# zilliztech/knowhere

Measured on AMD Instinct MI355X. Metric: QPS at recall@10>=0.95, IVF-PQ 100M x d=128 batch=10k, higher is better.
Workload: dtype f32

## Files before the change

### knowhere_amd/csrc/kernels.h

```cpp
#pragma once

#include <hip/hip_runtime.h>
#include <stdint.h>
#include <algorithm>
#include "sq_codec.h"

namespace knhip {

struct KnItem {
    int32_t list;
    int32_t npair;
    int64_t pair0;
};
struct KnPair {
    int32_t q;
    int32_t slot;
};

__host__ __device__ constexpr int pq_stream_phase(int lane) {
    const int l = lane & 31;
    return l < 4 ? l : l < 12 ? l + 4 : l < 16 ? l - 8 : l < 20 ? l - 16 : l < 28 ? l - 12 : l - 24;
}
constexpr int PQ_STREAM_PHASES = 16;
__host__ __device__ constexpr uint32_t pq_stream_mask(int j) {
    uint32_t m = 0;
    for (int l = 0; l < 32; l++) {
        if (pq_stream_phase(l) <= j) {
            m |= 1u << l;
        }
    }
    return m;
}
// ... 228 lines not shown
    P8Rec* pq_recs;
    const uint4* pq_codes_i;
    const void* pq_qi;
    const float* pq_qis;
    P16Rec* pq_recs16;
    int32_t* pq_ctr;
    int32_t pq_prune_mu;
    const void* pq_cb16;
    const void* pq_qh16;
    const float* pq_qd;
    const float* pq_sc;
    const float* pq_psum_s;
    unsigned char* pq_spill;
    int32_t pq_spill_cap;
    int32_t pq_spill_wgs;
    const int2* pq_unit_tiles;
};

int64_t pq_stream16r_blocks(int64_t len);
hipError_t launch_pq_stream16r(const uint8_t* codes, const int64_t* list_row_off, const int64_t* list_len,
                               const int64_t* list_sblk_off, int64_t nlist, uint4* out, hipStream_t s);
hipError_t launch_pq_psum(const uint8_t* codes, const int64_t* list_row_off, const int64_t* list_len,
                          const int64_t* list_sblk_off, int64_t nlist, const float* precomp_t, float* psum,
                          uint32_t* pabs_max_bits, hipStream_t s);
hipError_t launch_pqf_query_table(const float* queries, const float4* cb_m, int d, int64_t nq, bool is_l2, float pabs_max,
                                  void* qh, float* qs, hipStream_t s);
hipError_t launch_pqf_predict(const float* dump, int64_t stride, const int32_t* n_row, const float* gthr, const float* qs,
                              const float* qs2, const int64_t* keys, int nprobe, int64_t nlist, const int64_t* list_len,
                              int64_t nq, int cap, int k, bool is_l2, int32_t* poor, hipStream_t s);
size_t pqf_smem();
hipError_t launch_pq_stream16i(const uint8_t* codes, const int64_t* list_row_off, const int64_t* list_len,
// ... 60 lines not shown
hipError_t launch_pq_scan_q4(const PqScanArgs& a, bool is_l2, int64_t items_bound, hipStream_t s);
hipError_t launch_pq_cb_transpose(const float* cb, int M, int dsub, float4* cb_t, hipStream_t s);

int mscan_queries_per_unit(int kind, bool sample);
size_t mscan_flat_smem(int nstep);
size_t mscan_sq8_smem(int nstep, int bits = 8);
int mscan_finish_pmax(int cap, int k);
int mscan_sample_rows();
hipError_t launch_ms_block_norms(const float4* rows, int64_t total_blk, int nchunk, float* out, float* out_max,
                                 hipStream_t s, int row_type = KN_ROW_FP32);
hipError_t launch_ms_sq8_norms(const uint4* rows, int64_t total_blk, int nchunk16, int d, const float* trained,
                               float* out, float* out_max, hipStream_t s, int bits = 8);
hipError_t launch_ms_units(const int32_t* list_count_v, const int64_t* list_pair_off_v, int64_t nlist, int qt,
                           int64_t* unit_off, int64_t* nunits, KnItem* units, const int64_t* list_len,
                           int64_t code_size, double* unit_bytes, hipStream_t s, int cost_cap = 0,
                           int2* unit_tiles = nullptr);
inline int64_t ms_units_cost_bound(int64_t npairs, int qt, int64_t nlist, int64_t ntotal, int64_t max_len, int cost_cap) {
    const int64_t groups = npairs / qt + std::min<int64_t>(nlist, npairs) + 1;
    if (cost_cap <= 0) {
        return groups;
    }
    const int64_t max_ntile = std::max<int64_t>((max_len + 31) / 32, 1);
    const int64_t by_cost = groups + (2 * max_ntile * (npairs / 32 + groups) + cost_cap - 1) / cost_cap;
    const int64_t by_tiles = npairs / qt * max_ntile + ntotal / 32 + 2 * nlist + 1;
    return std::max<int64_t>(groups, std::min<int64_t>(by_cost, by_tiles));
}
hipError_t launch_mscan_flat(const MScanArgs& a, bool is_l2, int64_t units_bound, hipStream_t s);
int mscan_flat_bf16_qt(int nstep);
size_t mscan_flat_bf16_smem(int nstep);
hipError_t launch_mscan_flat_bf16(const MScanArgs& a, bool is_l2, int64_t units_bound, hipStream_t s);
hipError_t launch_mscan_sq8(const MScanArgs& a, bool is_l2, int64_t units_bound, hipStream_t s);
// ... 285 lines not shown
```

### knowhere_amd/csrc/knhip_api_search.hip

```cpp
#include "knhip_internal.h"

namespace knhip_host {

template <class A>
static A scan_args(const knhip_index* idx, const Workspace* ws, const Batch& b) {
    A a{};
    a.list_len = idx->d_list_len.as<int64_t>();
    a.list_row_off = idx->d_list_row_off.as<int64_t>();
    a.ids = idx->ids.as<int64_t>();
    a.d = idx->d;
    a.queries = b.q;
    a.bitset = b.bitset;
    a.bitset_nbits = b.nbits;
    a.partial_d = ws->partial_d.as<float>();
    a.partial_i = ws->partial_i.as<int64_t>();
    a.k = b.k;
    return a;
}
template <class A>
static A item_scan_args(const knhip_index* idx, const Workspace* ws, const Batch& b, const WorkTable& wt) {
    A a = scan_args<A>(idx, ws, b);
    a.items = wt.items;
    a.pairs = wt.pairs;
    a.nitems_dev = wt.nitems;
// ... 567 lines not shown
        HIP_TRY(ws->pq_recs16.reserve((size_t)std::max<int64_t>(std::max(plan.ms_units_bound, plan.ms_bound0), plan.npairs) *
                                      sizeof(P16Rec)));
        m.pq_codes_r = idx->rows_r.as<uint4>();
        m.pq_codes_i = idx->rows_i.as<uint4>();
        m.pq_qi = ws->ms_qi.p;
        m.pq_qis = ws->ms_qis.as<float>();
        m.pq_recs16 = ws->pq_recs16.as<P16Rec>();
    }
    if (f->form == 3) {
        f->qt = PD_QT;
        if (env.pqd_unit_cost > 0) {
            f->pqd_cost = env.pqd_unit_cost;
            f->pqd_bound = round_up(ms_units_cost_bound(plan.npairs, PD_QT, idx->nlist, idx->ntotal, idx->max_list_len,
                                                        f->pqd_cost), 8);
            HIP_TRY(ws->ms_units.reserve((size_t)f->pqd_bound * sizeof(KnItem)));
            HIP_TRY(ws->pqd_tiles.reserve((size_t)f->pqd_bound * sizeof(int2)));
            m.units = ws->ms_units.as<KnItem>();
            m.pq_unit_tiles = ws->pqd_tiles.as<int2>();
        }
        m.pq_cb16 = idx->pqd_cb16.p;
        m.pq_qh16 = ws->ms_qh16.p;
        m.pq_qd = ws->ms_qd.as<float>();
        m.pq_sc = idx->pqd_st.as<float>();
        m.pq_psum_s = idx->psum_s.as<float>();
        m.pq_spill_cap = 4 * 8192;
        if (idx->pqd_spill_cap > 0) {
            m.pq_spill_cap = idx->pqd_spill_cap;
        }
        m.pq_spill_wgs = 512;
        int dev = 0, ncu = 0;
        (void)hipGetDevice(&dev);
        if (hipDeviceGetAttribute(&ncu, hipDeviceAttributeMultiprocessorCount, dev) == hipSuccess && ncu > 0) {
            m.pq_spill_wgs = ncu;
// ... 93 lines not shown
}

int ms_group_units(const knhip_index* idx, Workspace* ws, const SearchPlan& plan, const Batch& b, const PqForm& f,
                   const WorkTable& wside, SideJoin* sj, hipStream_t s, MScanArgs& m) {
    const int64_t nlist = idx->nlist;
    StageTimer t(idx, s, KNHIP_STAGE_GROUP);
    if (sj->forked) {
        if (int rc = sj->join()) return rc;
    } else {
        HIP_TRY(launch_build_worktable(b.keys, b.nq, b.nprobe, nlist, plan.qg, plan.qg, idx->d_list_len.as<int64_t>(),
                                       idx->dev_code_size(), wside, s, -1));
    }
    m.pairs = wside.pairs;
    HIP_TRY(launch_ms_units(wside.list_count + nlist, wside.list_pair_off + nlist, nlist, f.qt, ws->ms_unit_off.as<int64_t>(),
                            ws->ms_nunits.as<int64_t>(), ws->ms_units.as<KnItem>(), idx->d_list_len.as<int64_t>(), idx->dev_code_size(),
                            idx->scan_bytes_dev.as<double>() + 2, s, f.pqd_cost, ws->pqd_tiles.as<int2>()));
    return KNHIP_OK;
}

int rows_exact_scan(const knhip_index* idx, Workspace* ws, const Batch& b, const WorkTable& wt, int64_t grid, bool one_pair,
                    hipStream_t s) {
    if (idx->desc.kind == KNHIP_IVF_FLAT) {
        FlatScanArgs a = flat_scan_args(idx, ws, b, wt);
        a.item_loop = one_pair;
        HIP_TRY(launch_flat_scan(a, idx->is_l2, false, grid, s, one_pair));
    } else {
        SqScanArgs a = sq_scan_args(idx, ws, b, wt);
        a.item_loop = one_pair;
        HIP_TRY(launch_sq_scan(a, idx->is_l2, grid, s, one_pair));
    }
    return KNHIP_OK;
// ... 30 lines not shown
    if (f.form == 2) {
        mf.pq_qs = m.pq_qis;
        mf.pq_prune_mu = 1;
    }
    if (f.form == 3) {
        mf.pq_qs = m.pq_qd;
    }
    HIP_TRY(launch_mscan_finish(mf, kind, is_l2, b.keys, b.cdis, nprobe, k, b.out_d, b.out_i, counters, 1, s));
    HIP_TRY(launch_ms_flag_pairs(m.overflow, 2, b.keys, nq, nprobe, nlist, idx->d_list_len.as<int64_t>(), k, wt.items, wt.pairs,
                                 wt.nitems, nullptr, s));
    MScanArgs r = m;
    r.pairs = wt.pairs;
    r.units = wt.items;
    r.nunits_dev = wt.nitems;
    r.unit_loop = 1;
    r.pq_unit_tiles = nullptr;
    r.ghist = nullptr;
    r.gmeta = nullptr;
    HIP_TRY(launch_filter(idx, plan, f, r, plan.npairs, s));
    HIP_TRY(launch_mscan_finish(mf, kind, is_l2, b.keys, b.cdis, nprobe, k, b.out_d, b.out_i, counters, 2, s));
    HIP_TRY(launch_ms_flag_pairs(m.overflow, 1, b.keys, nq, nprobe, nlist, idx->d_list_len.as<int64_t>(), k, wt.items, wt.pairs,
                                 wt.nitems, ws->partial_i.as<int64_t>(), s));
    if (int rc = exact_one_pair_items(idx, ws, plan, b, wt, s)) return rc;
    HIP_TRY(launch_merge_partials(ws->partial_d.as<float>(), ws->partial_i.as<int64_t>(), nq, nprobe, k, (int64_t)nprobe * k, k,
                                  is_l2, b.out_d, b.out_i, s, m.overflow));
    return KNHIP_OK;
}

int run_prefilter(const knhip_index* idx, Workspace* ws, const SearchPlan& plan, const Batch& b, const EnvSearch& env,
                  const WorkTable& wt, hipStream_t s, PqForm* f) {
    MScanArgs m;
// ... 155 lines not shown
```

### knowhere_amd/csrc/knhip_internal.h

```cpp
#pragma once
#include "../../include/knhip.h"
#include "common.h"
#include "kernels.h"
#include "knhip_env.h"

#include <cstdio>
#include <cstdlib>
#include <cstring>
#include <map>
#include <memory>
#include <mutex>
#include <numeric>
#include <random>
#include <string>
#include <vector>

using namespace knhip;

namespace knhip_host {

int fail(int code, const std::string& msg);

#define HIP_TRY(expr)                                                                              \
    do {                                                                                           \
// ... 100 lines not shown
    DevBuf recs4;
    DevBuf q4_ctr;
    DevBuf ghist;
    DevBuf gmeta;
    WorkTableBufs wt[2];
    DevBuf ms_qi, ms_qis, ms_qmu, pq_recs16;
    DevBuf rs_ovf;
    DevBuf ms_eps_max;
    DevBuf ms_cand_pess;
    DevBuf ms_units, ms_unit_off, ms_nunits, ms_cand, ms_cand_cnt;
    DevBuf ms_sample_off, ms_nrow;
    DevBuf ms_qh, ms_ql, ms_qs;
    DevBuf pq_recs, pq_ctr;
    DevBuf bf_kth;
    DevBuf ms_qh16, ms_qd, pq_spill;
    DevBuf pqd_tiles;
    DevBuf rs_sort;
    DevBuf h_queries, h_bitset, h_out_d, h_out_i, h_ref_d, h_ref_i;
    DevBuf tie_d, tie_i, tie_flag, tie_q, tie_r, tie_keys, tie_cdis;
    DevBuf tie_arr_d, tie_arr_i, tie_arr_n;
    DevBuf lk_plan, lk_scratch;
    std::mutex mu;
    hipStream_t side = nullptr;
    hipEvent_t ev_fork = nullptr, ev_join = nullptr;
    volatile int32_t* h_word = nullptr;
    int32_t word_seq = 0;
    ~Workspace() {
        if (h_word) (void)hipHostFree(const_cast<int32_t*>(h_word));
        if (ev_fork) (void)hipEventDestroy(ev_fork);
        if (ev_join) (void)hipEventDestroy(ev_join);
        if (side) (void)hipStreamDestroy(side);
// ... 262 lines not shown
```

### knowhere_amd/csrc/mfma_scan.hip

```cpp
#include "common.h"
#include "kernels.h"
#include "ms_common.h"

namespace knhip {

typedef float ms_f32x16 __attribute__((ext_vector_type(16)));
typedef _Float16 ms_f16x8 __attribute__((ext_vector_type(8)));

constexpr int MS_WAVES = 4;
constexpr int MS_THREADS = MS_WAVES * KN_WAVE;
constexpr int MS_NQT = 2;
constexpr int MS_QT = 32 * MS_NQT;
constexpr int MS_SAMPLE = 8192;

template <int RT = KN_ROW_FP32>
__global__ void ms_block_norms_kernel(const float4* __restrict__ rows, int64_t total_blk, int nchunk,
                                      float* __restrict__ out, float* __restrict__ out_max) {
    const int64_t t = (int64_t)blockIdx.x * blockDim.x + threadIdx.x;
    float acc = 0.f;
    if (t < total_blk * 64) {
        const int64_t b = t >> 6;
        const int r = (int)(t & 63);
        const float4* p = rows + b * (int64_t)nchunk * 64 + r;
        if constexpr (RT != KN_ROW_FP32) {
// ... 95 lines not shown
            }
            u += n[e];
        }
        carry += total;
        __syncthreads();
    }
    if (tid == 0) {
        unit_off[nlist] = carry;
        *nunits = carry;
    }
}

__global__ void ms_units_kernel(const int32_t* __restrict__ list_count_v, const int64_t* __restrict__ list_pair_off_v,
                                const int64_t* __restrict__ unit_off, int64_t nlist, int qt, KnItem* __restrict__ units,
                                const int64_t* __restrict__ list_len, int64_t code_size, double* unit_bytes, int cap,
                                int2* __restrict__ unit_tiles) {
    const int64_t l = (int64_t)blockIdx.x * blockDim.x + threadIdx.x;
    if (l >= nlist) {
        return;
    }
    const int64_t c = list_count_v[l];
    if (c > 0 && unit_bytes != nullptr) {
        atomicAdd(unit_bytes, (double)((c + qt - 1) / qt) * (double)list_len[l] * (double)code_size);
    }
    const int64_t p0 = list_pair_off_v[l];
    const int64_t ntile = cap > 0 ? (list_len[l] + 31) / 32 : 0;
    int64_t u = unit_off[l];
    for (int64_t i = 0; i < c; i += qt) {
        KnItem x;
        x.list = (int32_t)l;
        x.npair = (int32_t)min((int64_t)qt, c - i);
        x.pair0 = p0 + i;
        const int64_t nch = ms_group_chunks(ntile, x.npair, cap);
        for (int64_t j = 0; j < nch; j++, u++) {
            units[u] = x;
            if (cap > 0) {
                const int64_t t0 = j * ntile / nch, t1 = (j + 1) * ntile / nch;
                unit_tiles[u] = make_int2((int)t0, (int)(t1 - t0));
            }
        }
    }
}

hipError_t launch_ms_units(const int32_t* list_count_v, const int64_t* list_pair_off_v, int64_t nlist, int qt,
                           int64_t* unit_off, int64_t* nunits, KnItem* units, const int64_t* list_len,
                           int64_t code_size, double* unit_bytes, hipStream_t s, int cost_cap, int2* unit_tiles) {
    if (cost_cap > 0 && unit_tiles == nullptr) {
        return hipErrorInvalidValue;
    }
    hipLaunchKernelGGL(ms_unit_scan_kernel, dim3(1), dim3(MS_SCAN_THREADS), 0, s, list_count_v, nlist, qt, unit_off,
                       nunits, list_len, cost_cap);
    hipLaunchKernelGGL(ms_units_kernel, dim3((unsigned)((nlist + 255) / 256)), dim3(256), 0, s, list_count_v,
                       list_pair_off_v, unit_off, nlist, qt, units, list_len, code_size, unit_bytes, cost_cap, unit_tiles);
    return hipGetLastError();
}

template <int RT>
__device__ __forceinline__ float4 ms_row_operand(const float4& v, int hi) {
    if constexpr (RT == KN_ROW_FP32) {
        return v;
    } else {
        const uint32_t w0 = __float_as_uint(hi ? v.z : v.x), w1 = __float_as_uint(hi ? v.w : v.y);
        return make_float4(row_widen<RT>(w0 & 0xffffu), row_widen<RT>(w0 >> 16), row_widen<RT>(w1 & 0xffffu),
                           row_widen<RT>(w1 >> 16));
    }
}

template <bool IS_L2, bool DUMP, int NQT, int RT = KN_ROW_FP32>
// ... 1469 lines not shown
```

### knowhere_amd/csrc/ms_common.h

```cpp
#pragma once
#include "common.h"
#include "kernels.h"

namespace knhip {

template <bool IS_L2>
__device__ __forceinline__ void ms_emit(const MScanArgs& a, int32_t q, int32_t slot, int64_t row_off, int64_t pos,
                                        float pess) {
    if (a.bitset != nullptr && bitset_filtered(a.bitset, a.bitset_nbits, a.ids[row_off + pos])) {
        return;
    }
    const int n = atomicAdd(a.cand_cnt + q, 1);
    if (n < a.cap) {
        a.cand[(int64_t)q * a.cap + n] = ((int64_t)slot << 32) | (int64_t)(uint32_t)pos;
        if (a.cand_pess != nullptr) {
            a.cand_pess[(int64_t)q * a.cap + n] = pess;
        }
    } else {
        a.overflow[q] = 1;
        a.overflow[a.nq] = 1;
    }
    if (a.ghist != nullptr) {
        const uint2 mt = a.gmeta[q];
        if (mt.y != KN_HIST_OFF) {
// ... 43 lines not shown
            if (e == e && fabsf(e) < FLT_MAX) {
                bound = e;
            }
        }
    }
    return bound;
}

template <bool IS_L2>
__device__ __forceinline__ float ms_hist_bound(const MScanArgs& a, int32_t q, int k) {
    MsHist h;
    ms_hist_load(a, q, h);
    return ms_hist_eval<IS_L2>(h, k);
}

template <bool IS_L2>
__device__ __forceinline__ float ms_hist_bound_lane(const MScanArgs& a, int32_t q, int k) {
    float bound = worst_dist<IS_L2>();
    if (a.ghist == nullptr || q < 0) {
        return bound;
    }
    const uint2 mt = a.gmeta[q];
    if (mt.y == KN_HIST_OFF) {
        return bound;
    }
    const unsigned long long* hp = reinterpret_cast<const unsigned long long*>(a.ghist + (int64_t)q * KN_HIST_BINS);
    unsigned long long w[KN_HIST_BINS / 2];
#pragma unroll
    for (int i = 0; i < KN_HIST_BINS / 2; i++) {
        w[i] = __hip_atomic_load(hp + i, __ATOMIC_RELAXED, __HIP_MEMORY_SCOPE_AGENT);
// ... 33 lines not shown
```

### knowhere_amd/csrc/pq_decode.hip

```cpp
#include "common.h"
#include "kernels.h"
#include "ms_common.h"

#include <algorithm>
#include <cmath>
#include <cstdio>
#include <type_traits>

namespace knhip {

#ifndef PD_EXP
#define PD_EXP 0
#endif
constexpr int PD_M = 32;
constexpr int PD_KSUB = 256;
constexpr int PD_D = 128;
constexpr int PD_WAVES = 4;
constexpr int PD_THREADS = PD_WAVES * KN_WAVE;
constexpr int PD_CB_BYTES = PD_M * PD_KSUB * 8;
constexpr int PD_RING = 8;
constexpr int PD_REC_BYTES = 80;
constexpr int PD_REC_CAP = 176;
constexpr int PD_FLAT_CAP = 256;
constexpr int PD_PA_BYTES = PD_QT * 16;
constexpr int PD_W_PA = 0;
constexpr int PD_W_REC = PD_W_PA + 2 * PD_PA_BYTES;
constexpr int PD_W_FLAT = PD_W_REC + PD_REC_CAP * PD_REC_BYTES;
constexpr int PD_W_PCNT = PD_W_FLAT + PD_FLAT_CAP * 16;
constexpr int PD_W_CTL = PD_W_PCNT + 2 * PD_QT * 4;
constexpr int PD_W_BYTES = PD_W_CTL + 64;
constexpr int PD_OFF_W = PD_CB_BYTES;
constexpr int PD_SMEM = PD_OFF_W + PD_WAVES * PD_W_BYTES;
static_assert(PD_SMEM <= 160 * 1024, "LDS of one workgroup");
constexpr float PD_U = 5.9604645e-8f;
constexpr float PD_UH = 4.8828125e-4f;
constexpr float PD_A = 6.103515625e-5f;

#ifdef KNHIP_PHASE_TIMERS
#define PD_T(i)                                                         \
    do {                                                                \
        const unsigned long long t_ = __builtin_amdgcn_s_memtime();     \
        tacc[i] += t_ - tlast;                                          \
        tlast = t_;                                                     \
    } while (0)
#define PD_COUNT(i, n) tacc[i] += (unsigned long long)(n)
// ... 310 lines not shown
__device__ __forceinline__ void pd_ring_take(PdRing& r, pd_u4& w, float& p) {
    w = r.w[I];
    p = r.p[I];
}
__device__ __forceinline__ void pd_ring_drain(PdRing&) {}
#endif

__device__ __forceinline__ void pd_wave_sync() {
#if defined(__HIP_DEVICE_COMPILE__) && !defined(PD_NO_ASM)
    asm volatile("s_waitcnt lgkmcnt(0)" : : : "memory");
#else
    (void)__ballot(1);
#endif
}

struct PdUnit {
    int64_t len;
    int64_t row_off;
    int64_t ps_off;
    int ntile;
    uint32_t pos0;
};

template <bool IS_L2, int NTQ>
__device__ __forceinline__ int pqd_scan(const MScanArgs& a, unsigned char* smem, unsigned char* wb, const unsigned char* pa,
                                        int wslot, pd_h8 (&B)[4][8], const PdUnit& un PD_TARG) {
    const int lane = lane_id();
    const int lr = lane & 31, hi = lane >> 5;
    const float* sT = reinterpret_cast<const float*>(pa);
    const int32_t* sPq = reinterpret_cast<const int32_t*>(pa + 2 * PD_QT * 4);
    int32_t* ctl = reinterpret_cast<int32_t*>(wb + PD_W_CTL);
    unsigned char* rec = wb + PD_W_REC;
    const int ntile = un.ntile;
    const int spill_cap = a.pq_spill_cap / PD_WAVES;
    int nrec = 0;
    float sink = 0.f;
    bool wrote_global = false;

    float thr[NTQ];
#pragma unroll
    for (int qt = 0; qt < NTQ; qt++) {
// ... 242 lines not shown
        return;
    }
    const int lane = lane_id();
    const int wave = __builtin_amdgcn_readfirstlane((int)(threadIdx.x / KN_WAVE));
    const int wslot = (int)blockIdx.x * PD_WAVES + wave;
    unsigned char* wb = smem + PD_OFF_W + wave * PD_W_BYTES;
    int32_t* ctl = reinterpret_cast<int32_t*>(wb + PD_W_CTL);
    const int per = (nunits + 7) / 8;
    uint32_t xcc = 0;
    if (!LOOP) {
        asm volatile("s_getreg_b32 %0, hwreg(HW_REG_XCC_ID)" : "=s"(xcc));
    }
    const int xcd = (int)(xcc & 7u);
    int fetch_t = 0;
    int loop_u = wslot;
    auto fetch = [&]() -> int {
        int u = -1;
        if (LOOP) {
            u = loop_u < nunits ? loop_u : -1;
            loop_u += (int)gridDim.x * PD_WAVES;
            return u;
        }
        if (lane == 0) {
            while (fetch_t < 8) {
                const int x = (xcd + fetch_t) & 7;
                const int base = x * per;
                const int cnt = min(per, nunits - base);
                if (cnt > 0) {
                    const int i = atomicAdd(a.pq_ctr + x * 16, 1);
                    if (i < cnt) {
                        u = base + i;
                        break;
                    }
                }
                fetch_t++;
            }
        }
        return __builtin_amdgcn_readfirstlane(u);
    };
    {
        const uint4* src = reinterpret_cast<const uint4*>(a.pq_cb16);
        uint4* dst = reinterpret_cast<uint4*>(smem);
#pragma unroll 4
        for (int i = threadIdx.x; i < PD_CB_BYTES / 16; i += PD_THREADS) {
            dst[i] = src[i];
        }
    }
    int cur = fetch();
    int nxt = cur >= 0 ? fetch() : -1;
    __syncthreads();
    if (cur < 0) {
        return;
    }
    const float SC = a.pq_sc[6], inv_sc = a.pq_sc[7];
    auto pa_of = [&](int par) -> unsigned char* { return wb + PD_W_PA + par * PD_PA_BYTES; };
    struct Pairs2 {
        KnPair p[2];
    };
    auto pair_of = [&](int u) -> Pairs2 {
        Pairs2 r;
        r.p[0].q = r.p[1].q = -1;
        r.p[0].slot = r.p[1].slot = 0;
        if (u >= 0) {
            const KnItem it = a.units[u];
#pragma unroll
            for (int h = 0; h < 2; h++) {
                if (lane + 64 * h < it.npair) {
                    r.p[h] = a.pairs[it.pair0 + lane + 64 * h];
                }
            }
        }
        return r;
    };
    struct PairConst {
        float dis0[2], tau[2], epsb[2];
    };
    auto pair_request = [&](const Pairs2& pp, PairConst& pc) {
#pragma unroll
        for (int h = 0; h < 2; h++) {
            const KnPair p = pp.p[h];
            pc.dis0[h] = 0.f;
            pc.tau[h] = worst_dist<IS_L2>();
            pc.epsb[h] = INFINITY;
            if (p.q >= 0) {
                pc.dis0[h] = a.coarse_dis[(int64_t)p.q * a.nslot + p.slot];
                pc.tau[h] = tighter<IS_L2>(a.gthr[p.q], ms_hist_bound_lane<IS_L2>(a, p.q, a.k));
                pc.epsb[h] = a.pq_qd[(int64_t)p.q * 4 + 2];
            }
        }
    };
    auto pair_write = [&](const Pairs2& pp, const PairConst& pc, int par) {
        unsigned char* pa = pa_of(par);
#pragma unroll
        for (int h = 0; h < 2; h++) {
            const KnPair p = pp.p[h];
            const int pj = lane + 64 * h;
            float t = INFINITY, c = 0.f;
            if (p.q >= 0) {
                const float eps = pc.epsb[h] + 64.0f * PD_U * (fabsf(pc.dis0[h]) + fabsf(pc.tau[h]));
                if (pc.tau[h] == worst_dist<IS_L2>() || !(eps < INFINITY)) {
                    a.overflow[p.q] = 1;
                    a.overflow[a.nq] = 1;
                } else {
                    t = IS_L2 ? SC * (((pc.dis0[h] - pc.tau[h]) - eps) * 0.5f) : SC * ((pc.tau[h] - eps) - pc.dis0[h]);
                    c = IS_L2 ? pc.dis0[h] + eps : pc.dis0[h] - eps;
                }
            }
            reinterpret_cast<float*>(pa)[pj] = t;
            reinterpret_cast<float*>(pa + PD_QT * 4)[pj] = c;
            reinterpret_cast<int32_t*>(pa + 2 * PD_QT * 4)[pj] = p.q;
            reinterpret_cast<int32_t*>(pa + 3 * PD_QT * 4)[pj] = p.slot;
        }
    };
    pd_h8 B[4][8];
    auto load_queries = [&](int par, int ntq) {
        const int lr = lane & 31, hi = lane >> 5;
        const int32_t* sPq = reinterpret_cast<const int32_t*>(pa_of(par) + 2 * PD_QT * 4);
        const uint4* qh = reinterpret_cast<const uint4*>(a.pq_qh16);
#pragma unroll
        for (int qt = 0; qt < 4; qt++) {
            if (qt < ntq) {
                const int32_t q = sPq[qt * 32 + lr];
                const uint4* src = qh + ((int64_t)(q < 0 ? 0 : q) * (PD_D / 8) + hi * 8);
#pragma unroll
                for (int s = 0; s < 8; s++) {
                    const uint4 w = src[s];
                    B[qt][s] = __builtin_bit_cast(pd_h8, w);
                }
            }
        }
    };
    int par = 0;
    {
        const Pairs2 p0 = pair_of(cur);
        PairConst c0;
        pair_request(p0, c0);
        pair_write(p0, c0, 0);
    }
    Pairs2 pn = pair_of(nxt);
    pd_wave_sync();
    load_queries(0, (a.units[cur].npair + 31) >> 5);
    while (cur >= 0) {
        const KnItem it = a.units[cur];
        const int ntq = (it.npair + 31) >> 5;
        PdUnit un;
        {
            const int64_t llen = a.list_len[it.list];
            int t0 = 0, nt = (int)((llen + 31) >> 5);
            if (a.pq_unit_tiles != nullptr) {
                const int2 tr = a.pq_unit_tiles[cur];
                t0 = tr.x;
                nt = tr.y;
            }
            un.pos0 = 32u * (uint32_t)t0;
            un.len = min(llen - (int64_t)un.pos0, (int64_t)nt * 32);
            un.row_off = a.list_row_off[it.list] + un.pos0;
            un.ps_off = IS_L2 ? a.pq_sblk_off_r[it.list] * 16 + un.pos0 : 0;
            un.ntile = nt;
        }
        unsigned char* pa = pa_of(par);
        float* sT = reinterpret_cast<float*>(pa);
        float* sC = reinterpret_cast<float*>(pa + PD_QT * 4);
        int32_t* sPq = reinterpret_cast<int32_t*>(pa + 2 * PD_QT * 4);
        int32_t* sPs = reinterpret_cast<int32_t*>(pa + 3 * PD_QT * 4);
        int32_t* pcnt = reinterpret_cast<int32_t*>(wb + PD_W_PCNT);
        int32_t* pbase = pcnt + PD_QT;
        pcnt[lane] = 0;
        pcnt[lane + 64] = 0;
        if (lane == 0) {
            ctl[1] = 0;
            ctl[2] = 0;
        }
        pd_wave_sync();
        const int nn = nxt >= 0 ? fetch() : -1;
        PD_T(0);
        int nrec = 0;
        if (un.ntile > 0) {
            switch (ntq) {
                case 1: nrec = pqd_scan<IS_L2, 1>(a, smem, wb, pa, wslot, B, un PD_TPASS); break;
                case 2: nrec = pqd_scan<IS_L2, 2>(a, smem, wb, pa, wslot, B, un PD_TPASS); break;
                case 3: nrec = pqd_scan<IS_L2, 3>(a, smem, wb, pa, wslot, B, un PD_TPASS); break;
                default: nrec = pqd_scan<IS_L2, 4>(a, smem, wb, pa, wslot, B, un PD_TPASS); break;
            }
        }
        PD_T(2);
        PairConst cn;
        pair_request(pn, cn);
        pd_wave_sync();
        PD_T(4);
        uint4* flat = reinterpret_cast<uint4*>(wb + PD_W_FLAT);
        auto sort_out = [&](const uint32_t (&rw)[PD_REC_BYTES / 4]) {
            const uint32_t pair = rw[0], row0 = rw[1];
            const float thq = sT[pair];
            uint32_t hm = 0;
#pragma unroll
            for (int r = 0; r < 16; r++) {
                const uint32_t pos = row0 + (uint32_t)((r & 3) + 8 * (r >> 2));
                hm |= (__uint_as_float(rw[4 + r]) >= thq && (int64_t)pos < un.len) ? (1u << r) : 0u;
            }
            while (hm != 0u) {
                const int r = __ffs((int)hm) - 1;
                hm &= hm - 1u;
                uint32_t xb = rw[4];
#pragma unroll
                for (int r2 = 1; r2 < 16; r2++) {
                    xb = r == r2 ? rw[4 + r2] : xb;
                }
                const uint32_t pos = row0 + (uint32_t)((r & 3) + 8 * (r >> 2));
                if (a.bitset != nullptr && bitset_filtered(a.bitset, a.bitset_nbits, a.ids[un.row_off + (int64_t)pos])) {
                    continue;
                }
                const int at = atomicAdd(&ctl[1], 1);
                if (at < PD_FLAT_CAP) {
                    const int rank = atomicAdd(&pcnt[pair], 1);
                    flat[at] = make_uint4(pair, un.pos0 + pos, xb, (uint32_t)rank);
                } else {
                    const float xs = __uint_as_float(xb) * inv_sc, c = sC[pair];
                    ms_emit<IS_L2>(a, sPq[pair], sPs[pair], un.row_off - un.pos0, (int64_t)(un.pos0 + pos),
                                   IS_L2 ? c - 2.0f * xs : c + xs);
                }
            }
        };
        if (nrec > 0) {
            const int n_own = min(nrec, PD_REC_CAP), n_gl = min(ctl[2], a.pq_spill_cap / PD_WAVES);
            for (int i = lane; i < n_own; i += KN_WAVE) {
                uint32_t rw[PD_REC_BYTES / 4];
                const unsigned char* rp = wb + PD_W_REC + i * PD_REC_BYTES;
#pragma unroll
                for (int j = 0; j < PD_REC_BYTES / 16; j++) {
                    const uint4 q4 = reinterpret_cast<const uint4*>(rp)[j];
                    rw[4 * j] = q4.x;
                    rw[4 * j + 1] = q4.y;
                    rw[4 * j + 2] = q4.z;
// ... 12 lines not shown
                sort_out(rw);
            }
        }
        pair_write(pn, cn, par ^ 1);
        PD_T(3);
        pd_wave_sync();
#ifdef KNHIP_PHASE_TIMERS
        if (lane == 0) {
            atomicMax(&g_pd_prof[33], (unsigned long long)ctl[2]);
            atomicMax(&g_pd_prof[34], (unsigned long long)ctl[1]);
            atomicAdd(&g_pd_prof[35], (unsigned long long)nrec);
            atomicAdd(&g_pd_prof[36], (unsigned long long)ctl[1]);
            atomicAdd(&g_pd_prof[37], (unsigned long long)(ctl[2] > 0));
        }
#endif
        if (nxt >= 0) {
            load_queries(par ^ 1, (a.units[nxt].npair + 31) >> 5);
        }
        pn = pair_of(nn);
        const int nflat = min(ctl[1], PD_FLAT_CAP);
        if (nflat > 0) {
            static_assert(PD_FLAT_CAP == 4 * KN_WAVE, "four rows per lane");
            uint4 fe[4];
            uint2 mt[4];
#pragma unroll
            for (int b = 0; b < 4; b++) {
                const int i = lane + KN_WAVE * b;
                fe[b] = make_uint4(0u, 0u, 0u, 0u);
                mt[b] = make_uint2(0u, KN_HIST_OFF);
                if (i < nflat) {
                    fe[b] = flat[i];
                    if (a.ghist != nullptr) {
                        mt[b] = a.gmeta[sPq[fe[b].x]];
                    }
                }
            }
#pragma unroll
            for (int h = 0; h < 2; h++) {
                const int j = lane + 64 * h;
                const int c = pcnt[j];
                if (c > 0) {
                    const int32_t q = sPq[j];
                    const int base = atomicAdd(a.cand_cnt + q, c);
                    pbase[j] = base;
                    if (base + c > a.cap) {
                        a.overflow[q] = 1;
                        a.overflow[a.nq] = 1;
                    }
                }
            }
            pd_wave_sync();
#pragma unroll
            for (int b = 0; b < 4; b++) {
                const int i = lane + KN_WAVE * b;
                if (i < nflat) {
                    const uint4 h = fe[b];
                    const int32_t q = sPq[h.x];
                    const float x = __uint_as_float(h.z) * inv_sc, c = sC[h.x];
                    const float pess = IS_L2 ? c - 2.0f * x : c + x;
                    const int n = pbase[h.x] + (int)h.w;
// ... 28 lines not shown
    if (units_bound <= 0) {
        return hipSuccess;
    }
    if (a.dump != nullptr || a.pq_spill == nullptr || a.pq_spill_cap <= 0 || a.pq_cb16 == nullptr || a.pq_qh16 == nullptr || a.pq_qd == nullptr || a.pq_sc == nullptr ||
        a.pq_codes == nullptr || a.pq_ctr == nullptr || (is_l2 && (a.pq_psum_s == nullptr || a.pq_sblk_off_r == nullptr))) {
        return hipErrorInvalidValue;
    }
    int dev = 0, ncu = 0;
    (void)hipGetDevice(&dev);
    (void)hipDeviceGetAttribute(&ncu, hipDeviceAttributeMultiprocessorCount, dev);
    if (ncu <= 0) {
        ncu = 256;
    }
    auto kern = a.unit_loop ? (is_l2 ? pqd_kernel<true, true> : pqd_kernel<false, true>)
                            : (is_l2 ? pqd_kernel<true, false> : pqd_kernel<false, false>);
    hipError_t e = hipFuncSetAttribute(reinterpret_cast<const void*>(kern), hipFuncAttributeMaxDynamicSharedMemorySize,
                                       (int)PD_SMEM);
    if (e != hipSuccess) {
        return e;
    }
    if (!a.unit_loop) {
        e = hipMemsetAsync(a.pq_ctr, 0, 8 * 16 * sizeof(int32_t), s);
        if (e != hipSuccess) {
            return e;
        }
    }
    const int64_t grid = std::min<int64_t>(std::min<int64_t>((units_bound + PD_WAVES - 1) / PD_WAVES, ncu), a.pq_spill_wgs);
#ifdef KNHIP_PHASE_TIMERS
    static unsigned long long zero[40] = {0};
    (void)hipMemcpyToSymbol(HIP_SYMBOL(g_pd_prof), zero, sizeof(zero));
#endif
    hipLaunchKernelGGL(kern, dim3((unsigned)grid), dim3(PD_THREADS), PD_SMEM, s, a);
#ifdef KNHIP_PHASE_TIMERS
    (void)hipStreamSynchronize(s);
// ... 25 lines not shown
```

Baseline: 1.555 million.

## Precompute PQ decode unit descriptors and prefetch per-unit metadata ahead of use

The unit-building kernel now writes a 48-byte descriptor per unit (row offset, psum offset, pair range, tile range, length). The decode kernel double-buffers these descriptors in LDS instead of chasing units, list_len, list_row_off and sblk_off pointers inside the hot loop. The work-stealing atomic is split into issue and resolve so its latency overlaps the scan. Histogram rows are loaded early and evaluated later, candidate-count atomics and flat-entry loads are hoisted before the next query load, and the shared-memory attribute call is cached per device. These changes aim to hide global-memory latency and cut per-unit overhead, at the cost of more registers per lane and extra LDS per wave.

```diff
diff --git a/knowhere_amd/csrc/kernels.h b/knowhere_amd/csrc/kernels.h
--- a/knowhere_amd/csrc/kernels.h
+++ b/knowhere_amd/csrc/kernels.h
@@ -16,6 +16,18 @@
     int32_t q;
     int32_t slot;
 };
+struct alignas(16) PdUnitDesc {
+    int64_t row_off;
+    int64_t ps_off;
+    int64_t pair0;
+    int32_t len;
+    int32_t ntile;
+    uint32_t pos0;
+    int32_t npair;
+    int32_t list;
+    int32_t pad_;
+};
+static_assert(sizeof(PdUnitDesc) == 48, "three 16-byte words");
 
 __host__ __device__ constexpr int pq_stream_phase(int lane) {
     const int l = lane & 31;
@@ -274,7 +286,7 @@
     unsigned char* pq_spill;
     int32_t pq_spill_cap;
     int32_t pq_spill_wgs;
-    const int2* pq_unit_tiles;
+    const PdUnitDesc* pq_unit_desc;
 };
 
 int64_t pq_stream16r_blocks(int64_t len);
@@ -365,7 +377,8 @@
 hipError_t launch_ms_units(const int32_t* list_count_v, const int64_t* list_pair_off_v, int64_t nlist, int qt,
                            int64_t* unit_off, int64_t* nunits, KnItem* units, const int64_t* list_len,
                            int64_t code_size, double* unit_bytes, hipStream_t s, int cost_cap = 0,
-                           int2* unit_tiles = nullptr);
+                           PdUnitDesc* unit_desc = nullptr, const int64_t* list_row_off = nullptr,
+                           const int64_t* sblk_off = nullptr);
 inline int64_t ms_units_cost_bound(int64_t npairs, int qt, int64_t nlist, int64_t ntotal, int64_t max_len, int cost_cap) {
     const int64_t groups = npairs / qt + std::min<int64_t>(nlist, npairs) + 1;
     if (cost_cap <= 0) {
diff --git a/knowhere_amd/csrc/knhip_api_search.hip b/knowhere_amd/csrc/knhip_api_search.hip
--- a/knowhere_amd/csrc/knhip_api_search.hip
+++ b/knowhere_amd/csrc/knhip_api_search.hip
@@ -605,9 +605,9 @@
             f->pqd_bound = round_up(ms_units_cost_bound(plan.npairs, PD_QT, idx->nlist, idx->ntotal, idx->max_list_len,
                                                         f->pqd_cost), 8);
             HIP_TRY(ws->ms_units.reserve((size_t)f->pqd_bound * sizeof(KnItem)));
-            HIP_TRY(ws->pqd_tiles.reserve((size_t)f->pqd_bound * sizeof(int2)));
+            HIP_TRY(ws->pqd_desc.reserve((size_t)f->pqd_bound * sizeof(PdUnitDesc)));
             m.units = ws->ms_units.as<KnItem>();
-            m.pq_unit_tiles = ws->pqd_tiles.as<int2>();
+            m.pq_unit_desc = ws->pqd_desc.as<PdUnitDesc>();
         }
         m.pq_cb16 = idx->pqd_cb16.p;
         m.pq_qh16 = ws->ms_qh16.p;
@@ -731,7 +731,8 @@
     m.pairs = wside.pairs;
     HIP_TRY(launch_ms_units(wside.list_count + nlist, wside.list_pair_off + nlist, nlist, f.qt, ws->ms_unit_off.as<int64_t>(),
                             ws->ms_nunits.as<int64_t>(), ws->ms_units.as<KnItem>(), idx->d_list_len.as<int64_t>(), idx->dev_code_size(),
-                            idx->scan_bytes_dev.as<double>() + 2, s, f.pqd_cost, ws->pqd_tiles.as<int2>()));
+                            idx->scan_bytes_dev.as<double>() + 2, s, f.pqd_cost, ws->pqd_desc.as<PdUnitDesc>(), m.list_row_off,
+                            idx->is_l2 ? m.pq_sblk_off_r : nullptr));
     return KNHIP_OK;
 }
 
@@ -792,7 +793,7 @@
     r.units = wt.items;
     r.nunits_dev = wt.nitems;
     r.unit_loop = 1;
-    r.pq_unit_tiles = nullptr;
+    r.pq_unit_desc = nullptr;
     r.ghist = nullptr;
     r.gmeta = nullptr;
     HIP_TRY(launch_filter(idx, plan, f, r, plan.npairs, s));
diff --git a/knowhere_amd/csrc/knhip_internal.h b/knowhere_amd/csrc/knhip_internal.h
--- a/knowhere_amd/csrc/knhip_internal.h
+++ b/knowhere_amd/csrc/knhip_internal.h
@@ -138,7 +138,7 @@
     DevBuf pq_recs, pq_ctr;
     DevBuf bf_kth;
     DevBuf ms_qh16, ms_qd, pq_spill;
-    DevBuf pqd_tiles;
+    DevBuf pqd_desc;
     DevBuf rs_sort;
     DevBuf h_queries, h_bitset, h_out_d, h_out_i, h_ref_d, h_ref_i;
     DevBuf tie_d, tie_i, tie_flag, tie_q, tie_r, tie_keys, tie_cdis;
diff --git a/knowhere_amd/csrc/mfma_scan.hip b/knowhere_amd/csrc/mfma_scan.hip
--- a/knowhere_amd/csrc/mfma_scan.hip
+++ b/knowhere_amd/csrc/mfma_scan.hip
@@ -133,7 +133,8 @@
 __global__ void ms_units_kernel(const int32_t* __restrict__ list_count_v, const int64_t* __restrict__ list_pair_off_v,
                                 const int64_t* __restrict__ unit_off, int64_t nlist, int qt, KnItem* __restrict__ units,
                                 const int64_t* __restrict__ list_len, int64_t code_size, double* unit_bytes, int cap,
-                                int2* __restrict__ unit_tiles) {
+                                PdUnitDesc* __restrict__ unit_desc, const int64_t* __restrict__ list_row_off,
+                                const int64_t* __restrict__ sblk_off) {
     const int64_t l = (int64_t)blockIdx.x * blockDim.x + threadIdx.x;
     if (l >= nlist) {
         return;
@@ -143,7 +144,10 @@
         atomicAdd(unit_bytes, (double)((c + qt - 1) / qt) * (double)list_len[l] * (double)code_size);
     }
     const int64_t p0 = list_pair_off_v[l];
-    const int64_t ntile = cap > 0 ? (list_len[l] + 31) / 32 : 0;
+    const int64_t llen = cap > 0 ? list_len[l] : 0;
+    const int64_t ntile = (llen + 31) / 32;
+    const int64_t row0 = cap > 0 ? list_row_off[l] : 0;
+    const int64_t ps0 = (cap > 0 && sblk_off != nullptr) ? sblk_off[l] * 16 : 0;
     int64_t u = unit_off[l];
     for (int64_t i = 0; i < c; i += qt) {
         KnItem x;
@@ -155,7 +159,17 @@
             units[u] = x;
             if (cap > 0) {
                 const int64_t t0 = j * ntile / nch, t1 = (j + 1) * ntile / nch;
-                unit_tiles[u] = make_int2((int)t0, (int)(t1 - t0));
+                PdUnitDesc dsc;
+                dsc.pos0 = (uint32_t)(32 * t0);
+                dsc.ntile = (int32_t)(t1 - t0);
+                dsc.len = (int32_t)min(llen - 32 * t0, 32 * (t1 - t0));
+                dsc.row_off = row0 + 32 * t0;
+                dsc.ps_off = sblk_off != nullptr ? ps0 + 32 * t0 : 0;
+                dsc.pair0 = x.pair0;
+                dsc.npair = x.npair;
+                dsc.list = x.list;
+                dsc.pad_ = 0;
+                unit_desc[u] = dsc;
             }
         }
     }
@@ -163,14 +177,16 @@
 
 hipError_t launch_ms_units(const int32_t* list_count_v, const int64_t* list_pair_off_v, int64_t nlist, int qt,
                            int64_t* unit_off, int64_t* nunits, KnItem* units, const int64_t* list_len,
-                           int64_t code_size, double* unit_bytes, hipStream_t s, int cost_cap, int2* unit_tiles) {
-    if (cost_cap > 0 && unit_tiles == nullptr) {
+                           int64_t code_size, double* unit_bytes, hipStream_t s, int cost_cap, PdUnitDesc* unit_desc,
+                           const int64_t* list_row_off, const int64_t* sblk_off) {
+    if (cost_cap > 0 && (unit_desc == nullptr || list_row_off == nullptr)) {
         return hipErrorInvalidValue;
     }
     hipLaunchKernelGGL(ms_unit_scan_kernel, dim3(1), dim3(MS_SCAN_THREADS), 0, s, list_count_v, nlist, qt, unit_off,
                        nunits, list_len, cost_cap);
     hipLaunchKernelGGL(ms_units_kernel, dim3((unsigned)((nlist + 255) / 256)), dim3(256), 0, s, list_count_v,
-                       list_pair_off_v, unit_off, nlist, qt, units, list_len, code_size, unit_bytes, cost_cap, unit_tiles);
+                       list_pair_off_v, unit_off, nlist, qt, units, list_len, code_size, unit_bytes, cost_cap, unit_desc,
+                       list_row_off, sblk_off);
     return hipGetLastError();
 }
 
diff --git a/knowhere_amd/csrc/ms_common.h b/knowhere_amd/csrc/ms_common.h
--- a/knowhere_amd/csrc/ms_common.h
+++ b/knowhere_amd/csrc/ms_common.h
@@ -81,6 +81,60 @@
     return ms_hist_eval<IS_L2>(h, k);
 }
 
+typedef uint32_t ms_u4 __attribute__((ext_vector_type(4)));
+struct MsHistLane {
+    bool on;
+    uint2 mt;
+    ms_u4 w[KN_HIST_BINS / 4];
+};
+
+__device__ __forceinline__ void ms_hist_lane_load(const MScanArgs& a, int32_t q, MsHistLane& h) {
+    const uint64_t bytes = (uint64_t)a.nq * (KN_HIST_BINS * 4);
+    h.on = a.ghist != nullptr && q >= 0 && bytes <= 0xffffffffull;
+    h.mt = make_uint2(0u, KN_HIST_OFF);
+#pragma unroll
+    for (int i = 0; i < KN_HIST_BINS / 4; i++) {
+        h.w[i] = ms_u4{0u, 0u, 0u, 0u};
+    }
+    if (h.on) {
+        const __amdgpu_buffer_rsrc_t rs = __builtin_amdgcn_make_buffer_rsrc(a.ghist, 0, (int)(uint32_t)bytes, 0x00020000);
+        h.mt = a.gmeta[q];
+        const int off = (int)((uint32_t)q * (uint32_t)(KN_HIST_BINS * 4));
+#pragma unroll
+        for (int i = 0; i < KN_HIST_BINS / 4; i++) {
+            h.w[i] = __builtin_amdgcn_raw_buffer_load_b128(rs, off + 16 * i, 0,  16);
+        }
+    }
+}
+
+template <bool IS_L2>
+__device__ __forceinline__ float ms_hist_lane_eval(const MsHistLane& h, int k) {
+    float bound = worst_dist<IS_L2>();
+    if (!h.on || h.mt.y == KN_HIST_OFF) {
+        return bound;
+    }
+    uint32_t cum = 0;
+    int b = KN_HIST_BINS;
+#pragma unroll
+    for (int i = 0; i < KN_HIST_BINS / 4; i++) {
+#pragma unroll
+        for (int j = 0; j < 4; j++) {
+            cum += h.w[i][j];
+            b = (b == KN_HIST_BINS && cum >= (uint32_t)k) ? 4 * i + j : b;
+        }
+    }
+    if (b < KN_HIST_BINS - 1) {
+        const unsigned long long edge = (unsigned long long)h.mt.x + (((unsigned long long)b + 1ull) << h.mt.y) - 1ull;
+        if (edge < 0xffffffffull) {
+            const float e = dist_key_inv<IS_L2>((uint32_t)edge);
+            if (e == e && fabsf(e) < FLT_MAX) {
+                bound = e;
+            }
+        }
+    }
+    return bound;
+}
+
 template <bool IS_L2>
 __device__ __forceinline__ float ms_hist_bound_lane(const MScanArgs& a, int32_t q, int k) {
     float bound = worst_dist<IS_L2>();
diff --git a/knowhere_amd/csrc/pq_decode.hip b/knowhere_amd/csrc/pq_decode.hip
--- a/knowhere_amd/csrc/pq_decode.hip
+++ b/knowhere_amd/csrc/pq_decode.hip
@@ -3,6 +3,7 @@
 #include "ms_common.h"
 
 #include <algorithm>
+#include <atomic>
 #include <cmath>
 #include <cstdio>
 #include <type_traits>
@@ -28,7 +29,9 @@
 constexpr int PD_W_FLAT = PD_W_REC + PD_REC_CAP * PD_REC_BYTES;
 constexpr int PD_W_PCNT = PD_W_FLAT + PD_FLAT_CAP * 16;
 constexpr int PD_W_CTL = PD_W_PCNT + 2 * PD_QT * 4;
-constexpr int PD_W_BYTES = PD_W_CTL + 64;
+constexpr int PD_W_DESC = PD_W_CTL + 64;
+constexpr int PD_W_BYTES = PD_W_DESC + 2 * (int)sizeof(PdUnitDesc);
+static_assert(PD_W_DESC % 16 == 0 && PD_W_BYTES % 16 == 0, "16-byte LDS accesses");
 constexpr int PD_OFF_W = PD_CB_BYTES;
 constexpr int PD_SMEM = PD_OFF_W + PD_WAVES * PD_W_BYTES;
 static_assert(PD_SMEM <= 160 * 1024, "LDS of one workgroup");
@@ -369,17 +372,10 @@
 #endif
 }
 
-struct PdUnit {
-    int64_t len;
-    int64_t row_off;
-    int64_t ps_off;
-    int ntile;
-    uint32_t pos0;
-};
 
 template <bool IS_L2, int NTQ>
 __device__ __forceinline__ int pqd_scan(const MScanArgs& a, unsigned char* smem, unsigned char* wb, const unsigned char* pa,
-                                        int wslot, pd_h8 (&B)[4][8], const PdUnit& un PD_TARG) {
+                                        int wslot, pd_h8 (&B)[4][8], const PdUnitDesc& un PD_TARG) {
     const int lane = lane_id();
     const int lr = lane & 31, hi = lane >> 5;
     const float* sT = reinterpret_cast<const float*>(pa);
@@ -652,7 +648,17 @@
     const int xcd = (int)(xcc & 7u);
     int fetch_t = 0;
     int loop_u = wslot;
-    auto fetch = [&]() -> int {
+    auto fetch_issue = [&]() -> int {
+        int i = -1;
+        if (!LOOP && lane == 0 && fetch_t < 8) {
+            const int x = (xcd + fetch_t) & 7;
+            if (min(per, nunits - x * per) > 0) {
+                i = atomicAdd(a.pq_ctr + x * 16, 1);
+            }
+        }
+        return i;
+    };
+    auto fetch_resolve = [&](int i) -> int {
         int u = -1;
         if (LOOP) {
             u = loop_u < nunits ? loop_u : -1;
@@ -665,13 +671,16 @@
                 const int base = x * per;
                 const int cnt = min(per, nunits - base);
                 if (cnt > 0) {
-                    const int i = atomicAdd(a.pq_ctr + x * 16, 1);
+                    if (i < 0) {
+                        i = atomicAdd(a.pq_ctr + x * 16, 1);
+                    }
                     if (i < cnt) {
                         u = base + i;
                         break;
                     }
                 }
                 fetch_t++;
+                i = -1;
             }
         }
         return __builtin_amdgcn_readfirstlane(u);
@@ -684,8 +693,8 @@
             dst[i] = src[i];
         }
     }
-    int cur = fetch();
-    int nxt = cur >= 0 ? fetch() : -1;
+    int cur = fetch_resolve(fetch_issue());
+    int nxt = cur >= 0 ? fetch_resolve(fetch_issue()) : -1;
     __syncthreads();
     if (cur < 0) {
         return;
@@ -695,34 +704,66 @@
     struct Pairs2 {
         KnPair p[2];
     };
-    auto pair_of = [&](int u) -> Pairs2 {
+    auto desc_of = [&](int u) -> PdUnitDesc {
+        PdUnitDesc dsc;
+        dsc.row_off = dsc.ps_off = dsc.pair0 = 0;
+        dsc.len = dsc.ntile = dsc.npair = dsc.list = dsc.pad_ = 0;
+        dsc.pos0 = 0u;
+        if (u >= 0) {
+            if (a.pq_unit_desc != nullptr) {
+                dsc = a.pq_unit_desc[u];
+            } else {
+                const KnItem it = a.units[u];
+                const int64_t llen = a.list_len[it.list];
+                dsc.len = (int32_t)llen;
+                dsc.ntile = (int32_t)((llen + 31) >> 5);
+                dsc.row_off = a.list_row_off[it.list];
+                dsc.ps_off = IS_L2 ? a.pq_sblk_off_r[it.list] * 16 : 0;
+                dsc.pair0 = it.pair0;
+                dsc.npair = it.npair;
+                dsc.list = it.list;
+            }
+        }
+        return dsc;
+    };
+    auto desc_put = [&](int slot, const PdUnitDesc& dsc) {
+        if (lane == 0) {
+            *reinterpret_cast<PdUnitDesc*>(wb + PD_W_DESC + slot * (int)sizeof(PdUnitDesc)) = dsc;
+        }
+    };
+    auto desc_get = [&](int slot) -> PdUnitDesc {
+        PdUnitDesc dsc = *reinterpret_cast<const PdUnitDesc*>(wb + PD_W_DESC + slot * (int)sizeof(PdUnitDesc));
+        dsc.ntile = __builtin_amdgcn_readfirstlane(dsc.ntile);
+        dsc.npair = __builtin_amdgcn_readfirstlane(dsc.npair);
+        return dsc;
+    };
+    auto pair_of = [&](const PdUnitDesc& dsc) -> Pairs2 {
         Pairs2 r;
         r.p[0].q = r.p[1].q = -1;
         r.p[0].slot = r.p[1].slot = 0;
-        if (u >= 0) {
-            const KnItem it = a.units[u];
-#pragma unroll
-            for (int h = 0; h < 2; h++) {
-                if (lane + 64 * h < it.npair) {
-                    r.p[h] = a.pairs[it.pair0 + lane + 64 * h];
-                }
+#pragma unroll
+        for (int h = 0; h < 2; h++) {
+            if (lane + 64 * h < dsc.npair) {
+                r.p[h] = a.pairs[dsc.pair0 + lane + 64 * h];
             }
         }
         return r;
     };
     struct PairConst {
-        float dis0[2], tau[2], epsb[2];
+        float dis0[2], gthr[2], epsb[2];
+        MsHistLane hist[2];
     };
     auto pair_request = [&](const Pairs2& pp, PairConst& pc) {
 #pragma unroll
         for (int h = 0; h < 2; h++) {
             const KnPair p = pp.p[h];
             pc.dis0[h] = 0.f;
-            pc.tau[h] = worst_dist<IS_L2>();
+            pc.gthr[h] = worst_dist<IS_L2>();
             pc.epsb[h] = INFINITY;
+            ms_hist_lane_load(a, p.q, pc.hist[h]);
             if (p.q >= 0) {
                 pc.dis0[h] = a.coarse_dis[(int64_t)p.q * a.nslot + p.slot];
-                pc.tau[h] = tighter<IS_L2>(a.gthr[p.q], ms_hist_bound_lane<IS_L2>(a, p.q, a.k));
+                pc.gthr[h] = a.gthr[p.q];
                 pc.epsb[h] = a.pq_qd[(int64_t)p.q * 4 + 2];
             }
         }
@@ -735,12 +776,13 @@
             const int pj = lane + 64 * h;
             float t = INFINITY, c = 0.f;
             if (p.q >= 0) {
-                const float eps = pc.epsb[h] + 64.0f * PD_U * (fabsf(pc.dis0[h]) + fabsf(pc.tau[h]));
-                if (pc.tau[h] == worst_dist<IS_L2>() || !(eps < INFINITY)) {
+                const float tau = tighter<IS_L2>(pc.gthr[h], ms_hist_lane_eval<IS_L2>(pc.hist[h], a.k));
+                const float eps = pc.epsb[h] + 64.0f * PD_U * (fabsf(pc.dis0[h]) + fabsf(tau));
+                if (tau == worst_dist<IS_L2>() || !(eps < INFINITY)) {
                     a.overflow[p.q] = 1;
                     a.overflow[a.nq] = 1;
                 } else {
-                    t = IS_L2 ? SC * (((pc.dis0[h] - pc.tau[h]) - eps) * 0.5f) : SC * ((pc.tau[h] - eps) - pc.dis0[h]);
+                    t = IS_L2 ? SC * (((pc.dis0[h] - tau) - eps) * 0.5f) : SC * ((tau - eps) - pc.dis0[h]);
                     c = IS_L2 ? pc.dis0[h] + eps : pc.dis0[h] - eps;
                 }
             }
@@ -765,44 +807,33 @@
                     const uint4 w = src[s];
                     B[qt][s] = __builtin_bit_cast(pd_h8, w);
                 }
+            } else {
+#pragma unroll
+                for (int s = 0; s < 8; s++) {
+                    B[qt][s] = __builtin_bit_cast(pd_h8, make_uint4(0u, 0u, 0u, 0u));
+                }
             }
         }
     };
     int par = 0;
+    Pairs2 pn;
     {
-        const Pairs2 p0 = pair_of(cur);
+        const PdUnitDesc d0 = desc_of(cur), d1 = desc_of(nxt);
+        const Pairs2 p0 = pair_of(d0);
         PairConst c0;
         pair_request(p0, c0);
         pair_write(p0, c0, 0);
-    }
-    Pairs2 pn = pair_of(nxt);
+        pn = pair_of(d1);
+        desc_put(0, d0);
+        desc_put(1, d1);
+    }
     pd_wave_sync();
-    load_queries(0, (a.units[cur].npair + 31) >> 5);
+    load_queries(0, (desc_get(0).npair + 31) >> 5);
     while (cur >= 0) {
-        const KnItem it = a.units[cur];
-        const int ntq = (it.npair + 31) >> 5;
-        PdUnit un;
-        {
-            const int64_t llen = a.list_len[it.list];
-            int t0 = 0, nt = (int)((llen + 31) >> 5);
-            if (a.pq_unit_tiles != nullptr) {
-                const int2 tr = a.pq_unit_tiles[cur];
-                t0 = tr.x;
-                nt = tr.y;
-            }
-            un.pos0 = 32u * (uint32_t)t0;
-            un.len = min(llen - (int64_t)un.pos0, (int64_t)nt * 32);
-            un.row_off = a.list_row_off[it.list] + un.pos0;
-            un.ps_off = IS_L2 ? a.pq_sblk_off_r[it.list] * 16 + un.pos0 : 0;
-            un.ntile = nt;
-        }
+        const PdUnitDesc un = desc_get(par);
+        const int ntq = (un.npair + 31) >> 5;
         unsigned char* pa = pa_of(par);
-        float* sT = reinterpret_cast<float*>(pa);
-        float* sC = reinterpret_cast<float*>(pa + PD_QT * 4);
-        int32_t* sPq = reinterpret_cast<int32_t*>(pa + 2 * PD_QT * 4);
-        int32_t* sPs = reinterpret_cast<int32_t*>(pa + 3 * PD_QT * 4);
         int32_t* pcnt = reinterpret_cast<int32_t*>(wb + PD_W_PCNT);
-        int32_t* pbase = pcnt + PD_QT;
         pcnt[lane] = 0;
         pcnt[lane + 64] = 0;
         if (lane == 0) {
@@ -810,7 +841,7 @@
             ctl[2] = 0;
         }
         pd_wave_sync();
-        const int nn = nxt >= 0 ? fetch() : -1;
+        const int ticket = nxt >= 0 ? fetch_issue() : -1;
         PD_T(0);
         int nrec = 0;
         if (un.ntile > 0) {
@@ -822,6 +853,14 @@
             }
         }
         PD_T(2);
+        float* const sT = reinterpret_cast<float*>(pa);
+        float* const sC = reinterpret_cast<float*>(pa + PD_QT * 4);
+        int32_t* const sPq = reinterpret_cast<int32_t*>(pa + 2 * PD_QT * 4);
+        int32_t* const sPs = reinterpret_cast<int32_t*>(pa + 3 * PD_QT * 4);
+        int32_t* const pbase = pcnt + PD_QT;
+        const int nn = nxt >= 0 ? fetch_resolve(ticket) : -1;
+        const PdUnitDesc dnn = desc_of(nn);
+        const PdUnitDesc uf = desc_get(par);
         PairConst cn;
         pair_request(pn, cn);
         pd_wave_sync();
@@ -834,7 +873,7 @@
 #pragma unroll
             for (int r = 0; r < 16; r++) {
                 const uint32_t pos = row0 + (uint32_t)((r & 3) + 8 * (r >> 2));
-                hm |= (__uint_as_float(rw[4 + r]) >= thq && (int64_t)pos < un.len) ? (1u << r) : 0u;
+                hm |= (__uint_as_float(rw[4 + r]) >= thq && (int64_t)pos < uf.len) ? (1u << r) : 0u;
             }
             while (hm != 0u) {
                 const int r = __ffs((int)hm) - 1;
@@ -845,16 +884,16 @@
                     xb = r == r2 ? rw[4 + r2] : xb;
                 }
                 const uint32_t pos = row0 + (uint32_t)((r & 3) + 8 * (r >> 2));
-                if (a.bitset != nullptr && bitset_filtered(a.bitset, a.bitset_nbits, a.ids[un.row_off + (int64_t)pos])) {
+                if (a.bitset != nullptr && bitset_filtered(a.bitset, a.bitset_nbits, a.ids[uf.row_off + (int64_t)pos])) {
                     continue;
                 }
                 const int at = atomicAdd(&ctl[1], 1);
                 if (at < PD_FLAT_CAP) {
                     const int rank = atomicAdd(&pcnt[pair], 1);
-                    flat[at] = make_uint4(pair, un.pos0 + pos, xb, (uint32_t)rank);
+                    flat[at] = make_uint4(pair, uf.pos0 + pos, xb, (uint32_t)rank);
                 } else {
                     const float xs = __uint_as_float(xb) * inv_sc, c = sC[pair];
-                    ms_emit<IS_L2>(a, sPq[pair], sPs[pair], un.row_off - un.pos0, (int64_t)(un.pos0 + pos),
+                    ms_emit<IS_L2>(a, sPq[pair], sPs[pair], uf.row_off - uf.pos0, (int64_t)(uf.pos0 + pos),
                                    IS_L2 ? c - 2.0f * xs : c + xs);
                 }
             }
@@ -897,36 +936,45 @@
             atomicAdd(&g_pd_prof[37], (unsigned long long)(ctl[2] > 0));
         }
 #endif
+        const int nflat = __builtin_amdgcn_readfirstlane(min(ctl[1], PD_FLAT_CAP));
+        static_assert(PD_FLAT_CAP == 4 * KN_WAVE, "four rows per lane");
+        uint4 fe[4];
+        uint2 mt[4];
+        int rbase[2], rcnt[2];
+#pragma unroll
+        for (int h = 0; h < 2; h++) {
+            const int j = lane + 64 * h;
+            rcnt[h] = pcnt[j];
+            rbase[h] = 0;
+            if (rcnt[h] > 0) {
+                rbase[h] = atomicAdd(a.cand_cnt + sPq[j], rcnt[h]);
+            }
+        }
+#pragma unroll
+        for (int b = 0; b < 4; b++) {
+            const int i = lane + KN_WAVE * b;
+            fe[b] = make_uint4(0u, 0u, 0u, 0u);
+            mt[b] = make_uint2(0u, KN_HIST_OFF);
+            if (i < nflat) {
+                fe[b] = flat[i];
+                if (a.ghist != nullptr) {
+                    mt[b] = a.gmeta[sPq[fe[b].x]];
+                }
+            }
+        }
         if (nxt >= 0) {
-            load_queries(par ^ 1, (a.units[nxt].npair + 31) >> 5);
-        }
-        pn = pair_of(nn);
-        const int nflat = min(ctl[1], PD_FLAT_CAP);
+            load_queries(par ^ 1, (desc_get(par ^ 1).npair + 31) >> 5);
+        }
+        pn = pair_of(dnn);
+        desc_put(par, dnn);
         if (nflat > 0) {
-            static_assert(PD_FLAT_CAP == 4 * KN_WAVE, "four rows per lane");
-            uint4 fe[4];
-            uint2 mt[4];
-#pragma unroll
-            for (int b = 0; b < 4; b++) {
-                const int i = lane + KN_WAVE * b;
-                fe[b] = make_uint4(0u, 0u, 0u, 0u);
-                mt[b] = make_uint2(0u, KN_HIST_OFF);
-                if (i < nflat) {
-                    fe[b] = flat[i];
-                    if (a.ghist != nullptr) {
-                        mt[b] = a.gmeta[sPq[fe[b].x]];
-                    }
-                }
-            }
 #pragma unroll
             for (int h = 0; h < 2; h++) {
                 const int j = lane + 64 * h;
-                const int c = pcnt[j];
-                if (c > 0) {
-                    const int32_t q = sPq[j];
-                    const int base = atomicAdd(a.cand_cnt + q, c);
-                    pbase[j] = base;
-                    if (base + c > a.cap) {
+                if (rcnt[h] > 0) {
+                    pbase[j] = rbase[h];
+                    if (rbase[h] + rcnt[h] > a.cap) {
+                        const int32_t q = sPq[j];
                         a.overflow[q] = 1;
                         a.overflow[a.nq] = 1;
                     }
@@ -985,10 +1033,18 @@
     }
     auto kern = a.unit_loop ? (is_l2 ? pqd_kernel<true, true> : pqd_kernel<false, true>)
                             : (is_l2 ? pqd_kernel<true, false> : pqd_kernel<false, false>);
-    hipError_t e = hipFuncSetAttribute(reinterpret_cast<const void*>(kern), hipFuncAttributeMaxDynamicSharedMemorySize,
-                                       (int)PD_SMEM);
-    if (e != hipSuccess) {
-        return e;
+    constexpr int PD_MAX_DEV = 64;
+    static std::atomic<bool> attr_set[4][PD_MAX_DEV];
+    const int ki = (a.unit_loop ? 2 : 0) + (is_l2 ? 1 : 0);
+    hipError_t e = hipSuccess;
+    if (dev < 0 || dev >= PD_MAX_DEV || !attr_set[ki][dev].load(std::memory_order_acquire)) {
+        e = hipFuncSetAttribute(reinterpret_cast<const void*>(kern), hipFuncAttributeMaxDynamicSharedMemorySize, (int)PD_SMEM);
+        if (e != hipSuccess) {
+            return e;
+        }
+        if (dev >= 0 && dev < PD_MAX_DEV) {
+            attr_set[ki][dev].store(true, std::memory_order_release);
+        }
     }
     if (!a.unit_loop) {
         e = hipMemsetAsync(a.pq_ctr, 0, 8 * 16 * sizeof(int32_t), s);
```

Result: no change. 1.549 million, median of 2 (-0.4%).
